# kakao/buffalo

Measured on NVIDIA H100. Metric: interactions/sec (nnz/s) ALS d=128, higher is better.
Workload: dtype f32

## Files before the change

### buffalo_b200/csrc/als_tc.cuh

```cuda
#pragma once
#include "als_generic.cuh"
#include "bfl_common.cuh"
#include <type_traits>

#include "sm90_ptx.cuh"

namespace bfl {
namespace tc {

using namespace sm90;

constexpr int N_CONV = 4, KH = N_CONV / 4;
constexpr int W_EPI = 0, W_MMA = 4, W_CONV = 8, W_PLAN = W_CONV + N_CONV;
constexpr int WARPS = 16, THREADS = WARPS * 32;
constexpr int REG_MMA = 200, REG_PLAN = 4 * 128 - 128 - 128 - REG_MMA;
constexpr int NXS = 8;
constexpr int PT = 2;
constexpr int NS = 3;
constexpr int GATHER_AHEAD = 1;
constexpr int NPG = 8, NP = NPG * PT;
constexpr int NBV = 8;
template <int D>
struct Cfg {
    static constexpr int TILE = D == 128 ? 32 : 16;
    static constexpr int NF = D / 128;
    static constexpr int LBO = D * 16;
    static constexpr int OP_BYTES = TILE * D * 2;
};
constexpr uint32_t F_FIRST = 1u << 8, F_LAST = 1u << 9, F_NEG = 1u << 10, F_STOP = 1u << 11;

__device__ __forceinline__ int msw(int c) { return ((c >> 1) & 3) << 3; }

constexpr int G_FLOATS = 16 * 17 / 2 * 64;
__device__ __forceinline__ int g_block(int R, int C) { return (R * (R + 1) / 2 + C) * 64; }

template <int D>
union Stage {
    unsigned char op[PT][2][Cfg<D>::OP_BYTES];
    float raw[PT][Cfg<D>::TILE * D];
};
static_assert(sizeof(Stage<128>::op) == sizeof(Stage<128>::raw) && sizeof(Stage<256>::op) == sizeof(Stage<256>::raw),
              "a group's rows and its slabs fill the same stage");

template <int D>
struct Smem {
    static constexpr int TILE = Cfg<D>::TILE;
    alignas(1024) Stage<D> st[NS];
    alignas(128) float mat[128 * 128];
    alignas(16) float g[G_FLOATS];
    alignas(16) float bvec[NBV][KH][D];
    alignas(16) float sumq[NBV][KH][D];
    alignas(16) float xs[NXS][D];
    alignas(16) float pv[4][32];
    alignas(16) float dl[4][32];
    alignas(16) float sws[NP][TILE];
    alignas(16) float wv[NP][TILE];
    alignas(16) int32_t keys[NP][TILE];
    float wsum[NBV][KH];
    uint32_t meta_raw[NP];
    uint32_t meta_op[NS][PT];
    int badrow[NXS];
    alignas(8) uint64_t plan_full[NPG], plan_empty[NPG], raw_full[NS], op_full[NS], st_empty[NS];
    alignas(8) uint64_t acc_full, acc_empty, x_full[NXS], d_full[4];
};
template <int D>
struct SmemDet : Smem<D> {
    double lossp[NXS][4][2];
};
static_assert(sizeof(SmemDet<128>) <= 232448 && sizeof(SmemDet<256>) <= 232448, "shared memory of als_tc_kernel");

struct TcArgs {
    AlsArgs a;
    const int32_t* items;
    float* scratch;
    int64_t split;
    int pass;
    int debug;
};

template <int D>
__host__ __device__ constexpr size_t scratch_floats() { return (size_t)D * D + 2 * D + 4; }

__global__ void tc_absmax_kernel(const float* __restrict__ p, size_t n, unsigned int* __restrict__ out) {
    float m = 0.f;
    const size_t gtid = (size_t)blockIdx.x * blockDim.x + threadIdx.x, gsz = (size_t)gridDim.x * blockDim.x;
    const size_t lead = min(n, (size_t)(((16 - ((uintptr_t)p & 15)) & 15) / 4));
    const size_t n4 = (n - lead) / 4;
    const float4* p4 = reinterpret_cast<const float4*>(p + lead);
    for (size_t i = gtid; i < n4; i += gsz) {
        const float4 v = __ldg(p4 + i);
        m = fmaxf(fmaxf(m, fmaxf(fabsf(v.x), fabsf(v.y))), fmaxf(fabsf(v.z), fabsf(v.w)));
    }
    for (size_t i = gtid; i < lead; i += gsz) m = fmaxf(m, fabsf(p[i]));
    for (size_t i = lead + n4 * 4 + gtid; i < n; i += gsz) m = fmaxf(m, fabsf(p[i]));
    for (int o = 16; o > 0; o >>= 1) m = fmaxf(m, __shfl_xor_sync(FULL, m, o));
    if ((threadIdx.x & 31) == 0 && m > 0.f) atomicMax(out, __float_as_uint(m));
}
__global__ void tc_scale_kernel(const unsigned int* __restrict__ ymax, const unsigned int* __restrict__ vmax, float alpha,
                                float* __restrict__ out) {
    const float y = __uint_as_float(*ymax), w = __uint_as_float(*vmax) * fabsf(alpha);
    const float top = y * sqrtf(w);
    int e = 0;
    if (top > 0.f && isfinite(top)) {
        int ex;
        frexpf(top, &ex);
        e = 15 - ex;
    }
    e = max(-60, min(60, e));
    out[0] = ldexpf(1.f, e);
    out[1] = ldexpf(1.f, -2 * e);
}

template <int D, bool PARTIAL, bool LOSS1, bool DET = false>
__global__ void __launch_bounds__(THREADS, 1) als_tc_kernel(TcArgs ta) {
    static_assert(D == 128 || (D == 256 && PARTIAL), "fused row solve: d = 128; split-row mode: d = 128 or 256");
    constexpr int TILE = Cfg<D>::TILE, NF = Cfg<D>::NF, LBO = Cfg<D>::LBO;
    extern __shared__ __align__(1024) unsigned char smem_raw_[];
    Smem<D>& S = *reinterpret_cast<Smem<D>*>(smem_raw_);
    [[maybe_unused]] SmemDet<D>& SD = *reinterpret_cast<SmemDet<D>*>(smem_raw_);
    const AlsArgs& a = ta.a;
    const int tid = threadIdx.x, lane = tid & 31;
    const int warp = __shfl_sync(FULL, tid >> 5, 0);

    if (tid == 0) {
        for (int i = 0; i < NS; ++i) {
            mbar_init(&S.raw_full[i], N_CONV);
            mbar_init(&S.op_full[i], N_CONV);
            mbar_init(&S.st_empty[i], 4);
        }
        for (int i = 0; i < NPG; ++i) {
            mbar_init(&S.plan_full[i], 1);
            mbar_init(&S.plan_empty[i], N_CONV);
        }
        mbar_init(&S.acc_full, 4);
        mbar_init(&S.acc_empty, 4);
        for (int b = 0; b < 4; ++b) mbar_init(&S.d_full[b], 1);
        for (int i = 0; i < NXS; ++i) {
            mbar_init(&S.x_full[i], 4);
            S.badrow[i] = 0;
        }
        mbar_init_fence();
    }
    const float scale = __ldg(a.tc_scales), inv2 = __ldg(a.tc_scales + 1);
    if (!PARTIAL) {
        const float s2 = scale * scale;
        const bool zero = ta.debug & 32;
        for (int e = tid; e < 128 * 128; e += THREADS) {
            const int r = e >> 7, c = e & 127;
            if ((r >> 3) >= (c >> 3)) {
                float g = zero ? 0.f : __ldg(a.G + e);
                g += r == c && !zero ? a.reg : 0.f;
                S.g[g_block(r >> 3, c >> 3) + 8 * (r & 7) + (c & 7)] = g * s2;
            }
        }
    }
    __syncthreads();

    const int64_t nitems = a.row_end - a.row_begin;
    const int64_t my_first = (int64_t)blockIdx.x;
    const int64_t stride = gridDim.x;

    auto item_info = [&](int64_t it, int& row, int64_t& beg, int64_t& n, int& slot) {
        if (PARTIAL) {
            const int32_t* p = ta.items + 3 * (a.row_begin + it);
            row = p[0];
            const int64_t rb = row == 0 ? 0 : a.indptr[row - 1];
            const int64_t rn = a.indptr[row] - rb;
            beg = rb + (int64_t)p[1] * ta.split;
            n = min(ta.split, rn - (int64_t)p[1] * ta.split);
            slot = DET ? (int)it : p[2];
        } else {
            row = a.row_list[a.row_begin + it];
            beg = row == 0 ? 0 : a.indptr[row - 1];
            n = a.indptr[row] - beg;
            slot = 0;
        }
    };

    if (warp >= W_PLAN) {
        setmaxnreg_dec<REG_PLAN>();
        if (warp != W_PLAN) return;
        uint32_t gsl = 0, rph = 0, pe = 0;
        auto tile_begin = [&]() -> uint32_t {
            if (pe == 0) mbar_wait_idle(&S.plan_empty[gsl], rph ^ 1u);
            return gsl * PT + pe;
        };
        auto tile_end = [&]() {
            if (++pe == PT) {
                if (lane == 0) mbar_arrive(&S.plan_full[gsl]);
                pe = 0;
                if (++gsl == NPG) { gsl = 0; rph ^= 1u; }
            }
        };
        auto emit = [&](unsigned mask, uint32_t flags, int32_t key, float w) {
            const int cnt = __popc(mask);
            const int slot = __popc(mask & ((1u << lane) - 1u));
            const uint32_t rs = tile_begin();
            if ((mask >> lane) & 1u) {
                S.keys[rs][slot] = key;
                S.sws[rs][slot] = sqrtf(fabsf(w)) * scale;
                S.wv[rs][slot] = w;
            } else {
                const int zslot = cnt + lane - slot;
                if (zslot < TILE) {
                    S.sws[rs][zslot] = 0.f;
                    S.wv[rs][zslot] = 0.f;
                }
            }
            if (lane == 0) S.meta_raw[rs] = (uint32_t)cnt | flags;
            __syncwarp();
            tile_end();
        };
        constexpr int SC = 4, SCN = SC * TILE;
        const bool inl = lane < TILE;
        auto load_id = [&](int64_t it, int& row, int& chunk) {
            row = -1;
            chunk = 0;
            if (it < nitems) {
                if (PARTIAL) {
                    const int32_t* p = ta.items + 3 * (a.row_begin + it);
                    row = p[0];
                    chunk = p[1];
                } else {
                    row = a.row_list[a.row_begin + it];
                }
            }
        };
        auto load_span = [&](int row, int chunk, const int32_t*& kp, const float*& vp, int& n) {
            kp = a.keys;
            vp = a.vals;
            n = 0;
            if (row >= 0) {
                const int64_t rb = row == 0 ? 0 : a.indptr[row - 1];
                const int64_t rn = a.indptr[row] - rb;
                int64_t beg = rb;
                n = (int)rn;
                if (PARTIAL) {
                    beg = rb + (int64_t)chunk * ta.split;
                    n = (int)min(ta.split, rn - (int64_t)chunk * ta.split);
                }
                kp = a.keys + (beg - a.shift);
                vp = a.vals + (beg - a.shift);
            }
        };
        auto load_sc = [&](const int32_t* kp, const float* vp, int n, int c0, int32_t (&key)[SC], float (&w)[SC]) {
#pragma unroll
            for (int s = 0; s < SC; ++s) {
                const int idx = c0 + s * TILE + lane;
                const bool ok = inl && idx < n;
                key[s] = ok ? kp[idx] : 0;
                w[s] = ok ? vp[idx] * a.alpha : 0.f;
            }
        };
        auto emit_sc = [&](int n, int c0, const int32_t (&key)[SC], const float (&w)[SC]) {
            bool neg = false;
#pragma unroll
            for (int s = 0; s < SC; ++s) neg |= w[s] < 0.f;
            if (!__any_sync(FULL, neg)) {
#pragma unroll
                for (int s = 0; s < SC; ++s) {
                    const int t0 = c0 + s * TILE;
                    if (t0 < n) {
                        const uint32_t meta = (uint32_t)min(TILE, n - t0) | (t0 == 0 ? F_FIRST : 0u) | (t0 + TILE >= n ? F_LAST : 0u);
                        const uint32_t rs = tile_begin();
                        if (inl) {
                            float sq;
                            asm("sqrt.approx.ftz.f32 %0, %1;" : "=f"(sq) : "f"(w[s]));
                            S.keys[rs][lane] = key[s];
                            S.sws[rs][lane] = sq * scale;
                            S.wv[rs][lane] = w[s];
                        }
                        if (lane == 0) S.meta_raw[rs] = meta;
                        __syncwarp();
                        tile_end();
                    }
                }
            } else {
#pragma unroll
                for (int s = 0; s < SC; ++s) {
                    const int t0 = c0 + s * TILE;
                    if (t0 < n) {
                        const bool valid = inl && t0 + lane < n;
                        const unsigned pm = __ballot_sync(FULL, valid && !(w[s] < 0.f));
                        const unsigned nm = __ballot_sync(FULL, valid && (w[s] < 0.f));
                        const bool lastc = t0 + TILE >= n;
                        uint32_t fl = (t0 == 0 ? F_FIRST : 0u);
                        if (pm) {
                            emit(pm, fl | ((lastc && !nm) ? F_LAST : 0u), key[s], w[s]);
                            fl = 0u;
                        }
                        if (nm) emit(nm, fl | F_NEG | (lastc ? F_LAST : 0u), key[s], w[s]);
                    }
                }
            }
        };
        const int32_t *kp0, *kp1, *kp2, *kp3;
        const float *vp0, *vp1, *vp2, *vp3;
        int n0, n1, n2, n3;
        int row_t, ch_t, row4, ch4;
        int32_t k0[SC], k1[SC], k2[SC], nk[SC];
        float w0[SC], w1[SC], w2[SC], nw[SC];
        load_id(my_first, row_t, ch_t);
        load_span(row_t, ch_t, kp0, vp0, n0);
        load_sc(kp0, vp0, n0, 0, k0, w0);
        load_id(my_first + stride, row_t, ch_t);
        load_span(row_t, ch_t, kp1, vp1, n1);
        load_sc(kp1, vp1, n1, 0, k1, w1);
        load_id(my_first + 2 * stride, row_t, ch_t);
        load_span(row_t, ch_t, kp2, vp2, n2);
        load_id(my_first + 3 * stride, row4, ch4);
        for (int64_t it = my_first; it < nitems; it += stride) {
            load_sc(kp2, vp2, n2, 0, k2, w2);
            load_span(row4, ch4, kp3, vp3, n3);
            load_id(it + 4 * stride, row4, ch4);
            for (int c0 = 0; c0 < n0; c0 += SCN) {
                const bool more = c0 + SCN < n0;
                if (more) load_sc(kp0, vp0, n0, c0 + SCN, nk, nw);
                emit_sc(n0, c0, k0, w0);
                if (more) {
#pragma unroll
                    for (int s = 0; s < SC; ++s) { k0[s] = nk[s]; w0[s] = nw[s]; }
                }
            }
#pragma unroll
            for (int s = 0; s < SC; ++s) { k0[s] = k1[s]; w0[s] = w1[s]; k1[s] = k2[s]; w1[s] = w2[s]; }
            kp0 = kp1; vp0 = vp1; n0 = n1; kp1 = kp2; vp1 = vp2; n1 = n2; kp2 = kp3; vp2 = vp3; n2 = n3;
        }
        do {
            const uint32_t rs = tile_begin();
            if (lane == 0) S.meta_raw[rs] = F_STOP;
            __syncwarp();
            tile_end();
        } while (pe != 0);
    } else if (warp >= W_MMA && warp < W_MMA + 4) {
        setmaxnreg_inc<REG_MMA>();
        const int r0 = (D == 256 && ta.pass == 2) ? 128 : 0, c0 = (D == 256 && ta.pass > 0) ? 128 : 0;
        const int wq = warp - W_MMA;
        const int fr = 16 * wq + (lane >> 2), fc = 2 * (lane & 3);
        constexpr int N0 = PARTIAL ? 128 : 64;
        float d0[N0 / 2], d1[64];
        auto mma0 = [&](auto neg, uint64_t adesc, uint64_t bdesc) {
            constexpr bool NEG = decltype(neg)::value;
            if constexpr (PARTIAL) wgmma_m64n128k16_f16<NEG>(d0, adesc, bdesc);
            else wgmma_m64n64k16_f16<NEG>(d0, adesc, bdesc);
        };
        const int rb = 2 * wq;
        const int g_lo = 8 * (lane >> 2) + fc, g_up = 8 * fc + (lane >> 2);
        auto g_pair = [&](int R, int C) -> float2 {
            const bool low = R >= C;
            const float* p = S.g + (low ? g_block(R, C) + g_lo : g_block(C, R) + g_up);
            return make_float2(p[0], p[low ? 1 : 8]);
        };
        auto acc_init_nh = [&](const int n, const int h) {
            if constexpr (PARTIAL) {
                d0[4 * n + 2 * h] = 0.f; d0[4 * n + 2 * h + 1] = 0.f;
                d1[4 * n + 2 * h] = 0.f; d1[4 * n + 2 * h + 1] = 0.f;
            } else {
                if (8 * n < N0) {
                    const float2 g0 = g_pair(rb + h, n);
                    d0[4 * n + 2 * h] = g0.x; d0[4 * n + 2 * h + 1] = g0.y;
                }
                const float2 g1 = n < 8 ? *reinterpret_cast<const float2*>(S.g + g_block(8 + rb + h, n) + g_lo)
                                        : g_pair(8 + rb + h, n);
                d1[4 * n + 2 * h] = g1.x; d1[4 * n + 2 * h + 1] = g1.y;
            }
        };
        auto acc_init = [&]() {
#pragma unroll
            for (int n = 0; n < 16; ++n)
#pragma unroll
                for (int h = 0; h < 2; ++h) acc_init_nh(n, h);
        };
        uint32_t os = 0, oph = 0, aph = 0;
        int64_t seq = 0;
        bool stop = false;
        acc_init();
        while (!stop) {
            mbar_wait(&S.op_full[os], oph);
            fence_proxy_async_smem();
#pragma unroll 1
            for (int e = 0; e < PT; ++e) {
                const uint32_t meta = S.meta_op[os][e];
                if (meta & F_STOP) {
                    stop = true;
                    break;
                }
                const int ksteps = (ta.debug & 2) ? 0 : (int)(meta & 0xffu);
                const uint32_t hi = s32(&S.st[os].op[e][0][0]), lo = s32(&S.st[os].op[e][1][0]);
                wgmma_fence();
#pragma unroll 1
                for (int ks = 0; ks < ksteps; ++ks) {
                    const uint32_t k0 = ks * 2 * LBO;
                    const uint64_t ah0 = smem_desc(hi + k0 + r0 * 16, LBO, 128), ah1 = smem_desc(hi + k0 + (r0 + 64) * 16, LBO, 128);
                    const uint64_t al0 = smem_desc(lo + k0 + r0 * 16, LBO, 128), al1 = smem_desc(lo + k0 + (r0 + 64) * 16, LBO, 128);
                    const uint64_t bh = smem_desc(hi + k0 + c0 * 16, LBO, 128), bl = smem_desc(lo + k0 + c0 * 16, LBO, 128);
                    if (meta & F_NEG) {
                        mma0(std::true_type{}, ah0, bh);
                        mma0(std::true_type{}, ah0, bl);
                        mma0(std::true_type{}, al0, bh);
                        wgmma_m64n128k16_f16<true>(d1, ah1, bh);
                        wgmma_m64n128k16_f16<true>(d1, ah1, bl);
                        wgmma_m64n128k16_f16<true>(d1, al1, bh);
                    } else {
                        mma0(std::false_type{}, ah0, bh);
                        mma0(std::false_type{}, ah0, bl);
                        mma0(std::false_type{}, al0, bh);
                        wgmma_m64n128k16_f16<false>(d1, ah1, bh);
                        wgmma_m64n128k16_f16<false>(d1, ah1, bl);
                        wgmma_m64n128k16_f16<false>(d1, al1, bh);
                    }
                }
                wgmma_commit();
                if (meta & F_LAST) {
                    wgmma_wait<0>();
#pragma unroll
                    for (int i = 0; i < 64; ++i) { if (i < N0 / 2) acc_fence(d0[i]); acc_fence(d1[i]); }
                    mbar_wait_idle(&S.acc_empty, aph ^ 1u);
                    if constexpr (PARTIAL) {
                        const int slot = DET ? (int)(my_first + seq * stride) : ta.items[3 * (a.row_begin + my_first + seq * stride) + 2];
                        float* sc = ta.scratch + (size_t)slot * scratch_floats<D>();
#pragma unroll
                        for (int n = 0; n < 16; ++n)
#pragma unroll
                            for (int h = 0; h < 2; ++h)
#pragma unroll
                                for (int i = 0; i < 2; ++i) {
                                    const int r = r0 + fr + 8 * h, c = c0 + 8 * n + fc + i;
                                    const float v0 = d0[4 * n + 2 * h + i] * inv2, v1 = d1[4 * n + 2 * h + i] * inv2;
                                    if constexpr (DET) {
                                        sc[(size_t)r * D + c] = v0;
                                        sc[(size_t)(r + 64) * D + c] = v1;
                                        if (r0 != c0) {
                                            sc[(size_t)c * D + r] = v0;
                                            sc[(size_t)c * D + r + 64] = v1;
                                        }
                                    } else {
                                        atomicAdd(sc + (size_t)r * D + c, v0);
                                        atomicAdd(sc + (size_t)(r + 64) * D + c, v1);
                                        if (r0 != c0) {
                                            atomicAdd(sc + (size_t)c * D + r, v0);
                                            atomicAdd(sc + (size_t)c * D + r + 64, v1);
                                        }
                                    }
                                }
                        acc_init();
                    } else {
#pragma unroll
                        for (int n = 0; n < 16; ++n)
#pragma unroll
                            for (int h = 0; h < 2; ++h) {
#pragma unroll
                                for (int i = 0; i < 2; ++i) {
                                    const int r = fr + 8 * h, c = 8 * n + fc + i;
                                    const float v1 = d1[4 * n + 2 * h + i] * inv2;
                                    S.mat[c * 128 + ((r + 64) ^ msw(c))] = v1;
                                    if (8 * n < N0) {
                                        S.mat[c * 128 + (r ^ msw(c))] = d0[4 * n + 2 * h + i] * inv2;
                                        S.mat[(r + 64) * 128 + (c ^ msw(r + 64))] = v1;
                                    }
                                }
                                acc_init_nh(n, h);
                            }
                    }
                    __syncwarp();
                    if (lane == 0) mbar_arrive(&S.acc_full);
                    aph ^= 1u;
                    ++seq;
                }
            }
            wgmma_wait<0>();
#pragma unroll
            for (int i = 0; i < 64; ++i) { if (i < N0 / 2) acc_fence(d0[i]); acc_fence(d1[i]); }
            __syncwarp();
            if (lane == 0) mbar_arrive(&S.st_empty[os]);
            if (++os == NS) { os = 0; oph ^= 1u; }
        }
    } else if (warp >= W_CONV && warp < W_CONV + N_CONV) {
        const int cta = tid - W_CONV * 32;
        const int ct = cta & 127;
        const int kh = cta >> 7;
        constexpr int CHS = TILE / 8 / KH;
        uint32_t rs = 0, rph = 0, bslot = 0;
        float2 bacc[NF], qacc[NF];
        float wacc = 0.f;
#pragma unroll
        for (int f = 0; f < NF; ++f) { bacc[f] = make_float2(0.f, 0.f); qacc[f] = make_float2(0.f, 0.f); }
        const int cw = cta >> 5;
        uint32_t gs = 0, gph = 0, grs = 0, grph = 0;
        bool plan_end = false;
        auto gather = [&]() {
            if (plan_end) {
                cp_async_commit();
                return;
            }
            mbar_wait(&S.plan_full[gs], gph);
            mbar_wait(&S.st_empty[grs], grph ^ 1u);
            const uint32_t gm0 = S.meta_raw[gs * PT], gm1 = S.meta_raw[gs * PT + 1];
            if (PT == 2 && !(ta.debug & 1) && ((gm0 | gm1) & F_STOP) == 0 && (gm0 & 0xffu) == TILE && (gm1 & 0xffu) == TILE) {
                int32_t kk[PT][TILE / N_CONV];
#pragma unroll
                for (int e = 0; e < PT; ++e)
#pragma unroll
                    for (int i = 0; i < TILE / N_CONV; ++i) kk[e][i] = S.keys[gs * PT + e][cw + N_CONV * i];
#pragma unroll
                for (int e = 0; e < PT; ++e)
#pragma unroll
                    for (int i = 0; i < TILE / N_CONV; ++i) {
                        const float* src = a.Y + (int64_t)kk[e][i] * a.ld + lane * 4;
                        float* dst = &S.st[grs].raw[e][(cw + N_CONV * i) * D + lane * 4];
#pragma unroll
                        for (int c = 0; c < D / 128; ++c) cp_async16_cg(dst + c * 128, src + c * 128);
                    }
            } else
#pragma unroll
            for (int e = 0; e < PT; ++e) {
                const uint32_t gmeta = S.meta_raw[gs * PT + e];
                if (gmeta & F_STOP) {
                    plan_end = true;
                } else {
                    const int gcnt = (ta.debug & 1) ? 0 : (int)(gmeta & 0xffu);
#pragma unroll
                    for (int i = 0; i < TILE / N_CONV; ++i) {
                        const int slot = cw + N_CONV * i;
                        if (slot < gcnt) {
                            const float* src = a.Y + (int64_t)S.keys[gs * PT + e][slot] * a.ld + lane * 4;
                            float* dst = &S.st[grs].raw[e][slot * D + lane * 4];
#pragma unroll
                            for (int c = 0; c < D / 128; ++c) cp_async16_cg(dst + c * 128, src + c * 128);
                        }
                    }
                }
            }
            cp_async_commit();
            if (++gs == NPG) { gs = 0; gph ^= 1u; }
            if (++grs == NS) { grs = 0; grph ^= 1u; }
        };
        uint32_t cs = 0;
        bool done = false;
        if (ta.debug & 16) {
            uint32_t ph = 0;
            for (;;) {
                mbar_wait(&S.plan_full[cs], ph);
                const bool stop = (S.meta_raw[cs * PT] | S.meta_raw[cs * PT + 1]) & F_STOP;
                __syncwarp();
                if (lane == 0) mbar_arrive(&S.plan_empty[cs]);
                if (stop) break;
                if (++cs == NPG) { cs = 0; ph ^= 1u; }
            }
            if (cta == 0) S.meta_op[0][0] = F_STOP;
            __syncwarp();
            if (lane == 0) mbar_arrive(&S.op_full[0]);
            done = true;
        }
#pragma unroll 1
        for (int i = 0; i < GATHER_AHEAD && !done; ++i) gather();
        while (!done) {
            gather();
            cp_async_wait_group<GATHER_AHEAD>();
            __syncwarp();
            if (lane == 0) mbar_arrive(&S.raw_full[rs]);
            mbar_wait(&S.raw_full[rs], rph);
            float qv[PT][CHS * 8 * NF];
#pragma unroll
            for (int e = 0; e < PT; ++e)
#pragma unroll
                for (int c = 0; c < CHS; ++c)
#pragma unroll
                    for (int i = 0; i < 8; ++i)
#pragma unroll
                        for (int f = 0; f < NF; ++f)
                            qv[e][(c * 8 + i) * NF + f] = S.st[rs].raw[e][((kh * CHS + c) * 8 + i) * D + ct + 128 * f];
            named_bar_sync(1, N_CONV * 32);
            const uint32_t cm0 = S.meta_raw[cs * PT], cm1 = S.meta_raw[cs * PT + 1];
            const bool fast2 = PT == 2 && !(ta.debug & 4) && ((cm0 | cm1) & F_STOP) == 0 && (cm0 & 0xffu) == TILE &&
                               (cm1 & 0xffu) == TILE;
            if (fast2) {
#pragma unroll
                for (int e = 0; e < PT; ++e) {
                    const uint32_t meta = e == 0 ? cm0 : cm1;
                    const uint32_t psl = cs * PT + e;
                    const bool first = (meta & F_FIRST) != 0;
#pragma unroll
                    for (int f = 0; f < NF; ++f) {
                        bacc[f].x = first ? 0.f : bacc[f].x; bacc[f].y = first ? 0.f : bacc[f].y;
                        qacc[f].x = first ? 0.f : qacc[f].x; qacc[f].y = first ? 0.f : qacc[f].y;
                    }
                    wacc = first ? 0.f : wacc;
                    unsigned char* hi = &S.st[rs].op[e][0][0];
                    unsigned char* lo = &S.st[rs].op[e][1][0];
#pragma unroll
                    for (int c = 0; c < CHS; ++c) {
                        const int kc = kh * CHS + c, k0 = kc * 8;
                        const float4 sa = *reinterpret_cast<const float4*>(&S.sws[psl][k0]);
                        const float4 sb = *reinterpret_cast<const float4*>(&S.sws[psl][k0 + 4]);
                        const float4 wa = *reinterpret_cast<const float4*>(&S.wv[psl][k0]);
                        const float4 wb = *reinterpret_cast<const float4*>(&S.wv[psl][k0 + 4]);
                        if (LOSS1) wacc += ((wa.x + wa.y) + (wa.z + wa.w)) + ((wb.x + wb.y) + (wb.z + wb.w));
#pragma unroll
                        for (int f = 0; f < NF; ++f) {
                            const int m = ct + 128 * f;
                            const float* q = &qv[e][0];
                            const float2 q01 = make_float2(q[(c * 8 + 0) * NF + f], q[(c * 8 + 1) * NF + f]);
                            const float2 q23 = make_float2(q[(c * 8 + 2) * NF + f], q[(c * 8 + 3) * NF + f]);
                            const float2 q45 = make_float2(q[(c * 8 + 4) * NF + f], q[(c * 8 + 5) * NF + f]);
                            const float2 q67 = make_float2(q[(c * 8 + 6) * NF + f], q[(c * 8 + 7) * NF + f]);
                            uint4 h4, l4;
                            split_f16x2(f2mul(q01, make_float2(sa.x, sa.y)), h4.x, l4.x);
                            split_f16x2(f2mul(q23, make_float2(sa.z, sa.w)), h4.y, l4.y);
                            split_f16x2(f2mul(q45, make_float2(sb.x, sb.y)), h4.z, l4.z);
                            split_f16x2(f2mul(q67, make_float2(sb.z, sb.w)), h4.w, l4.w);
                            const int off = kc * LBO + (m >> 3) * 128 + (m & 7) * 16;
                            *reinterpret_cast<uint4*>(hi + off) = h4;
                            *reinterpret_cast<uint4*>(lo + off) = l4;
                            bacc[f] = f2fma(make_float2(wa.x, wa.y), q01, bacc[f]);
                            bacc[f] = f2fma(make_float2(wa.z, wa.w), q23, bacc[f]);
                            bacc[f] = f2fma(make_float2(wb.x, wb.y), q45, bacc[f]);
                            bacc[f] = f2fma(make_float2(wb.z, wb.w), q67, bacc[f]);
                            if (LOSS1) {
                                qacc[f].x += (q01.x + q23.x) + (q45.x + q67.x);
                                qacc[f].y += (q01.y + q23.y) + (q45.y + q67.y);
                            }
                        }
                    }
#pragma unroll
                    for (int f = 0; f < NF; ++f) {
                        S.bvec[bslot][kh][ct + 128 * f] = bacc[f].x + bacc[f].y;
                        if (LOSS1) S.sumq[bslot][kh][ct + 128 * f] = qacc[f].x + qacc[f].y;
                    }
                    if (LOSS1 && ct == 0) S.wsum[bslot][kh] = wacc;
                    bslot = (bslot + ((meta & F_LAST) ? 1u : 0u)) & (NBV - 1);
                    if (cta == 0) S.meta_op[rs][e] = (uint32_t)(TILE / 16) | (meta & (F_FIRST | F_LAST | F_NEG));
                }
            } else
#pragma unroll
            for (int e = 0; e < PT; ++e) {
                if (done) continue;
                const uint32_t psl = cs * PT + e;
                const uint32_t meta = S.meta_raw[psl];
                if (meta & F_STOP) {
                    if (cta == 0) S.meta_op[rs][e] = F_STOP;
                    done = true;
                    continue;
                }
                const int cnt = (int)(meta & 0xffu), ksteps = (cnt + 15) >> 4;
                if (meta & F_FIRST) {
#pragma unroll
                    for (int f = 0; f < NF; ++f) { bacc[f] = make_float2(0.f, 0.f); qacc[f] = make_float2(0.f, 0.f); }
                    wacc = 0.f;
                }
                unsigned char* hi = &S.st[rs].op[e][0][0];
                unsigned char* lo = &S.st[rs].op[e][1][0];
                auto chunk = [&](auto guard, const int c) {
                    constexpr bool GUARD = decltype(guard)::value;
                    const int kc = kh * CHS + c, k0 = kc * 8;
                    const float4 sa = *reinterpret_cast<const float4*>(&S.sws[psl][k0]);
                    const float4 sb = *reinterpret_cast<const float4*>(&S.sws[psl][k0 + 4]);
                    const float4 wa = *reinterpret_cast<const float4*>(&S.wv[psl][k0]);
                    const float4 wb = *reinterpret_cast<const float4*>(&S.wv[psl][k0 + 4]);
                    if (LOSS1) wacc += ((wa.x + wa.y) + (wa.z + wa.w)) + ((wb.x + wb.y) + (wb.z + wb.w));
#pragma unroll
                    for (int f = 0; f < NF; ++f) {
                        const int m = ct + 128 * f;
                        float q[8];
#pragma unroll
                        for (int i = 0; i < 8; ++i) q[i] = qv[e][(c * 8 + i) * NF + f];
                        if (GUARD) {
#pragma unroll
                            for (int i = 0; i < 8; ++i) q[i] = (k0 + i < cnt) ? q[i] : 0.f;
                        }
                        const float2 q01 = make_float2(q[0], q[1]), q23 = make_float2(q[2], q[3]);
                        const float2 q45 = make_float2(q[4], q[5]), q67 = make_float2(q[6], q[7]);
                        uint4 h4, l4;
                        split_f16x2(f2mul(q01, make_float2(sa.x, sa.y)), h4.x, l4.x);
                        split_f16x2(f2mul(q23, make_float2(sa.z, sa.w)), h4.y, l4.y);
                        split_f16x2(f2mul(q45, make_float2(sb.x, sb.y)), h4.z, l4.z);
                        split_f16x2(f2mul(q67, make_float2(sb.z, sb.w)), h4.w, l4.w);
                        const int off = kc * LBO + (m >> 3) * 128 + (m & 7) * 16;
                        *reinterpret_cast<uint4*>(hi + off) = h4;
                        *reinterpret_cast<uint4*>(lo + off) = l4;
                        bacc[f] = f2fma(make_float2(wa.x, wa.y), q01, bacc[f]);
                        bacc[f] = f2fma(make_float2(wa.z, wa.w), q23, bacc[f]);
                        bacc[f] = f2fma(make_float2(wb.x, wb.y), q45, bacc[f]);
                        bacc[f] = f2fma(make_float2(wb.z, wb.w), q67, bacc[f]);
                        if (LOSS1) {
                            qacc[f].x += (q[0] + q[2]) + (q[4] + q[6]);
                            qacc[f].y += (q[1] + q[3]) + (q[5] + q[7]);
                        }
                    }
                };
                if (ta.debug & 4) {
                } else if (cnt == TILE) {
#pragma unroll
                    for (int c = 0; c < CHS; ++c) chunk(std::false_type{}, c);
                } else {
#pragma unroll
                    for (int c = 0; c < CHS; ++c)
                        if (kh * CHS + c < 2 * ksteps) chunk(std::true_type{}, c);
                }
                if (meta & F_LAST) {
#pragma unroll
                    for (int f = 0; f < NF; ++f) {
                        S.bvec[bslot][kh][ct + 128 * f] = bacc[f].x + bacc[f].y;
                        if (LOSS1) S.sumq[bslot][kh][ct + 128 * f] = qacc[f].x + qacc[f].y;
                    }
                    if (LOSS1 && ct == 0) S.wsum[bslot][kh] = wacc;
                    bslot = (bslot + 1) & (NBV - 1);
                }
                if (cta == 0) S.meta_op[rs][e] = (uint32_t)ksteps | (meta & (F_FIRST | F_LAST | F_NEG));
            }
            __syncwarp();
            if (lane == 0) {
                mbar_arrive(&S.plan_empty[cs]);
                mbar_arrive(&S.op_full[rs]);
            }
            cs = (cs + 1) & (NPG - 1);
            if (++rs == NS) { rs = 0; rph ^= 1u; }
        }
    } else {
        const int q = warp & 3;
        const int j = q * 32 + lane;
        float* pv = S.pv[q];
        double l_nume = 0.0, l_deno = 0.0;
        const float tol = a.tol;
        if constexpr (PARTIAL) {
            int row = 0, slot = 0, nrow = 0, nslot = 0;
            int64_t beg, n = 0, nbeg, nn = 0;
            if (my_first < nitems) item_info(my_first, row, beg, n, slot);
            for (int64_t seq = 0; my_first + seq * stride < nitems; ++seq) {
                const int64_t nit = my_first + (seq + 1) * stride;
                if (nit < nitems) item_info(nit, nrow, nbeg, nn, nslot);
                const uint32_t aph = (uint32_t)(seq & 1);
                const uint32_t bs = (uint32_t)(seq & (NBV - 1));
                mbar_wait_idle(&S.acc_full, aph);
                float* sc = ta.scratch + (size_t)slot * scratch_floats<D>();
                if constexpr (DET) {
                    if (ta.pass == 0) {
                        for (int jj = j; jj < D; jj += 128) {
                            sc[(size_t)D * D + jj] = S.bvec[bs][0][jj] + (KH == 2 ? S.bvec[bs][KH - 1][jj] : 0.f);
                            if (LOSS1) sc[(size_t)D * D + D + jj] = S.sumq[bs][0][jj] + (KH == 2 ? S.sumq[bs][KH - 1][jj] : 0.f);
                        }
                        if (LOSS1 && j < 4)
                            sc[(size_t)D * D + 2 * D + j] = j == 0 ? S.wsum[bs][0] + (KH == 2 ? S.wsum[bs][KH - 1] : 0.f) : 0.f;
                    }
                } else if (ta.pass == 0) {
                    for (int jj = j; jj < D; jj += 128) {
                        atomicAdd(sc + (size_t)D * D + jj, S.bvec[bs][0][jj] + (KH == 2 ? S.bvec[bs][KH - 1][jj] : 0.f));
                        if (LOSS1) atomicAdd(sc + (size_t)D * D + D + jj, S.sumq[bs][0][jj] + (KH == 2 ? S.sumq[bs][KH - 1][jj] : 0.f));
                    }
                    if (LOSS1 && j == 0) atomicAdd(sc + (size_t)D * D + 2 * D, S.wsum[bs][0] + (KH == 2 ? S.wsum[bs][KH - 1] : 0.f));
                }
                __syncwarp();
                if (lane == 0) mbar_arrive(&S.acc_empty);
                row = nrow; slot = nslot; n = nn;
            }
        } else {
            auto row_of = [&](int64_t sq) -> int {
                const int64_t it = my_first + sq * stride;
                return it < nitems ? a.row_list[a.row_begin + it] : -1;
            };
            auto len_of = [&](int row) -> float {
                if (row < 0 || !a.compute_loss) return 0.f;
                return (float)(a.indptr[row] - (row == 0 ? 0 : a.indptr[row - 1]));
            };
            int row = (ta.debug & 16) ? -1 : row_of(0), row1 = row_of(1), row2 = row_of(2);
            float xj = row >= 0 ? a.X[(int64_t)row * a.ld + j] : 0.f;
            float x1 = row1 >= 0 ? a.X[(int64_t)row1 * a.ld + j] : 0.f;
            float nlen = len_of(row), nlen1 = len_of(row1);
            if (row >= 0) {
                S.xs[0][j] = xj;
                __syncwarp();
                if (lane == 0) mbar_arrive(&S.x_full[0]);
            }
            auto mat = [&](int c) -> float { return S.mat[c * 128 + (j ^ msw(c))]; };
            for (int64_t seq = 0; row >= 0; ++seq) {
                const int row3 = row_of(seq + 3);
                const float x2 = row2 >= 0 ? a.X[(int64_t)row2 * a.ld + j] : 0.f;
                const float nlen2 = len_of(row2);
                if (row1 >= 0) {
                    S.xs[(seq + 1) & (NXS - 1)][j] = x1;
                    __syncwarp();
                    if (lane == 0) mbar_arrive(&S.x_full[(seq + 1) & (NXS - 1)]);
                }
                const uint32_t aph = (uint32_t)(seq & 1);
                const uint32_t bs = (uint32_t)(seq & (NBV - 1));
                const uint32_t xsl = (uint32_t)(seq & (NXS - 1));
                const float* xs = S.xs[xsl];
                mbar_wait(&S.x_full[xsl], (uint32_t)((seq / NXS) & 1));
                mbar_wait_idle(&S.acc_full, aph);
                if (ta.debug & 8) {
                    __syncwarp();
                    if (lane == 0) mbar_arrive(&S.acc_empty);
                    row = row1; row1 = row2; row2 = row3;
                    xj = x1; x1 = x2;
                    continue;
                }
                const float bj = S.bvec[bs][0][j] + (KH == 2 ? S.bvec[bs][KH - 1][j] : 0.f);
                double ln_row = 0.0, ld_row = 0.0;
                float hM = 0.f;
                float md[32];
#pragma unroll
                for (int c = 0; c < D / 32; ++c) {
                    float h0 = 0.f, h1 = 0.f;
#pragma unroll
                    for (int i = 0; i < 32; i += 4) {
                        const float4 x4 = *reinterpret_cast<const float4*>(xs + c * 32 + i);
                        const float m0 = mat(c * 32 + i), m1 = mat(c * 32 + i + 1), m2 = mat(c * 32 + i + 2), m3 = mat(c * 32 + i + 3);
                        h0 = fmaf(m0, x4.x, h0); h1 = fmaf(m1, x4.y, h1);
                        h0 = fmaf(m2, x4.z, h0); h1 = fmaf(m3, x4.w, h1);
                        if (c == q) { md[i] = m0; md[i + 1] = m1; md[i + 2] = m2; md[i + 3] = m3; }
                    }
                    hM += h0 + h1;
                }
                if (a.compute_loss) {
                    const float kappa = a.adaptive_reg ? nlen : 1.0f;
                    double t = (double)(kappa * a.reg * xj * xj);
                    if (a.axis == 1) {
                        t += (double)xj * (double)hM - (double)(a.reg * xj * xj) -
                             2.0 * (double)xj * ((double)bj + (double)S.sumq[bs][0][j] + (KH == 2 ? (double)S.sumq[bs][KH - 1][j] : 0.0));
                        if (j == 0) {
                            const double ws = (double)S.wsum[bs][0] + (KH == 2 ? (double)S.wsum[bs][KH - 1] : 0.0);
                            t += (double)nlen + ws;
                            l_deno += (double)a.Y_rows + ws;
                        }
                    }
                    if constexpr (DET) {
                        ln_row = warp_sum_d(t);
                        ld_row = l_deno;
                        l_deno = 0.0;
                        if (q < 3 && lane == 0) {
                            SD.lossp[xsl][q][0] = ln_row;
                            SD.lossp[xsl][q][1] = ld_row;
                        }
                    } else {
                        l_nume += t;
                    }
                }
                float h = hM - bj;
#pragma unroll 1
                for (int B = 0; B < q; ++B) {
                    float mv[32];
#pragma unroll
                    for (int i = 0; i < 32; ++i) mv[i] = mat(B * 32 + i);
                    mbar_wait(&S.d_full[B], aph);
                    float u0 = 0.f, u1 = 0.f;
#pragma unroll
                    for (int i = 0; i < 32; i += 4) {
                        const float4 d4 = *reinterpret_cast<const float4*>(&S.dl[B][i]);
                        u0 = fmaf(mv[i], d4.x, u0);
                        u1 = fmaf(mv[i + 1], d4.y, u1);
                        u0 = fmaf(mv[i + 2], d4.z, u0);
                        u1 = fmaf(mv[i + 3], d4.w, u1);
                    }
                    h -= u0 + u1;
                }
                if constexpr (DET) {
                    if (q == 3 && lane == 0 && a.loss && a.compute_loss) {
                        double sn = SD.lossp[xsl][0][0], sd = SD.lossp[xsl][0][1];
#pragma unroll
                        for (int w = 1; w < 3; ++w) {
                            sn += SD.lossp[xsl][w][0];
                            sd += SD.lossp[xsl][w][1];
                        }
                        a.loss[2 * (int64_t)row] = sn + ln_row;
                        a.loss[2 * (int64_t)row + 1] = sd + ld_row;
                    }
                }
                __syncwarp();
                if (lane == 0) mbar_arrive(&S.acc_empty);
                float xv = 0.f;
                {
                    float r = h, p = h;
                    float rsold = warp_sum(r * r);
                    bool act = rsold > tol;
#pragma unroll 1
                    for (int step = 0; step < 3; ++step) {
                        pv[lane] = p;
                        __syncwarp();
                        float a0 = 0.f, a1 = 0.f, a2 = 0.f, a3 = 0.f;
#pragma unroll
                        for (int i = 0; i < 32; i += 4) {
                            const float4 p4 = *reinterpret_cast<const float4*>(pv + i);
                            a0 = fmaf(md[i], p4.x, a0); a1 = fmaf(md[i + 1], p4.y, a1);
                            a2 = fmaf(md[i + 2], p4.z, a2); a3 = fmaf(md[i + 3], p4.w, a3);
                        }
                        __syncwarp();
                        const float Ap = (a0 + a1) + (a2 + a3);
                        const float pAp = warp_sum(p * Ap);
                        const float ss = act ? __fdividef(rsold, pAp) : 0.f;
                        xv = fmaf(ss, p, xv);
                        r = fmaf(-ss, Ap, r);
                        const float rsnew = warp_sum(r * r);
                        act = act && !(rsnew < tol);
                        if (act) p = fmaf(__fdividef(rsnew, rsold), p, r);
                        rsold = act ? rsnew : rsold;
                    }
                }
                float v = xj - xv;
                const bool badw = __any_sync(FULL, !isfinite(v));
                a.X[(int64_t)row * a.ld + j] = v;
                for (int pr = 0; pr < a.n_peer; ++pr) a.peerX[pr][(int64_t)row * a.ld + j] = v;
                if (q < 3) {
                    S.dl[q][lane] = xv;
                    if (badw && lane == 0) atomicOr(&S.badrow[xsl], 1);
                    __syncwarp();
                    if (lane == 0) mbar_arrive(&S.d_full[q]);
                }
                if (q == 3) {
                    const bool bad = badw || (S.badrow[xsl] != 0);
                    if (bad) {
#pragma unroll
                        for (int c = 0; c < 4; ++c) {
                            a.X[(int64_t)row * a.ld + c * 32 + lane] = 0.f;
                            for (int pr = 0; pr < a.n_peer; ++pr) a.peerX[pr][(int64_t)row * a.ld + c * 32 + lane] = 0.f;
                        }
                        __syncwarp();
                        if (lane == 0) S.badrow[xsl] = 0;
                    }
                }
                row = row1; row1 = row2; row2 = row3;
                xj = x1; x1 = x2;
                nlen = nlen1; nlen1 = nlen2;
            }
            if (!DET && a.loss && a.compute_loss) {
                l_nume = warp_sum_d(l_nume);
                l_deno = warp_sum_d(l_deno);
                if (lane == 0 && (l_nume != 0.0 || l_deno != 0.0)) {
                    atomicAdd(a.loss, l_nume);
                    atomicAdd(a.loss + 1, l_deno);
                }
            }
        }
    }
}

inline bool tc_applicable(int optimizer_code, int d, int vdim, int block_size) {
    return optimizer_code == 8 && d == 128 && vdim == 128 && block_size == 32;
}
inline bool tc_split_applicable(int optimizer_code, int d, int vdim, int block_size) {
    return optimizer_code == 8 && (d == 128 || d == 256) && vdim == d && block_size == 32;
}

inline int tc_note_absmax(const float* p, size_t n, unsigned int* out, int num_sms, cudaStream_t st) {
    BFL_CUDA(cudaMemsetAsync(out, 0, sizeof(unsigned int), st));
    if (n == 0) return BFL_OK;
    const int grid = (int)std::min<size_t>((n / 4 + 255) / 256 + 1, (size_t)num_sms * 8);
    tc_absmax_kernel<<<grid, 256, 0, st>>>(p, n, out);
    BFL_LAUNCHED();
    return BFL_OK;
}
inline int tc_update_scale(const unsigned int* ymax, const unsigned int* vmax, float alpha, float* scales, cudaStream_t st) {
    tc_scale_kernel<<<1, 1, 0, st>>>(ymax, vmax, alpha, scales);
    BFL_LAUNCHED();
    return BFL_OK;
}

__global__ void tc_count_items_kernel(const int64_t* __restrict__ indptr, const int32_t* __restrict__ list, int64_t nrows,
                                      int64_t split, unsigned long long* total) {
    for (int64_t i = (int64_t)blockIdx.x * blockDim.x + threadIdx.x; i < nrows; i += (int64_t)gridDim.x * blockDim.x) {
        const int row = list[i];
        const int64_t n = indptr[row] - (row == 0 ? 0 : indptr[row - 1]);
        atomicAdd(total, (unsigned long long)((n + split - 1) / split));
    }
}
__global__ void tc_fill_items_kernel(const int64_t* __restrict__ indptr, const int32_t* __restrict__ list, int64_t nrows,
                                     int64_t split, unsigned long long* cursor, int32_t* __restrict__ items) {
    for (int64_t i = (int64_t)blockIdx.x * blockDim.x + threadIdx.x; i < nrows; i += (int64_t)gridDim.x * blockDim.x) {
        const int row = list[i];
        const int64_t n = indptr[row] - (row == 0 ? 0 : indptr[row - 1]);
        const int64_t nc = (n + split - 1) / split;
        const unsigned long long pos = atomicAdd(cursor, (unsigned long long)nc);
        for (int64_t c = 0; c < nc; ++c) {
            items[3 * (pos + c) + 0] = row;
            items[3 * (pos + c) + 1] = (int32_t)c;
            items[3 * (pos + c) + 2] = (int32_t)i;
        }
    }
}

__global__ void tc_chunk_counts_kernel(const int64_t* __restrict__ indptr, const int32_t* __restrict__ list, int64_t nrows,
                                       int64_t split, long long* __restrict__ counts) {
    for (int64_t i = (int64_t)blockIdx.x * blockDim.x + threadIdx.x; i < nrows; i += (int64_t)gridDim.x * blockDim.x) {
        const int row = list[i];
        const int64_t n = indptr[row] - (row == 0 ? 0 : indptr[row - 1]);
        counts[i] = (n + split - 1) / split;
    }
}
__global__ void tc_fill_items_scanned_kernel(const int32_t* __restrict__ list, int64_t nrows,
                                             const long long* __restrict__ chunk_end, int32_t* __restrict__ items) {
    for (int64_t i = (int64_t)blockIdx.x * blockDim.x + threadIdx.x; i < nrows; i += (int64_t)gridDim.x * blockDim.x) {
        const int64_t pos = i == 0 ? 0 : chunk_end[i - 1], nc = chunk_end[i] - pos;
        for (int64_t c = 0; c < nc; ++c) {
            items[3 * (pos + c) + 0] = list[i];
            items[3 * (pos + c) + 1] = (int32_t)c;
            items[3 * (pos + c) + 2] = (int32_t)i;
        }
    }
}

__global__ void __launch_bounds__(256) tc_chunk_reduce_kernel(const float* __restrict__ chunks, const long long* __restrict__ chunk_end,
                                                              int64_t row0, int64_t chunk0, size_t slot_floats, int nf4,
                                                              float* __restrict__ rows_out) {
    const int64_t i = row0 + blockIdx.y;
    const int64_t c0 = (i == 0 ? 0 : chunk_end[i - 1]) - chunk0, c1 = chunk_end[i] - chunk0;
    float4* out = reinterpret_cast<float4*>(rows_out + (size_t)blockIdx.y * slot_floats);
    for (int e = blockIdx.x * blockDim.x + threadIdx.x; e < nf4; e += gridDim.x * blockDim.x) {
        float4 acc = __ldg(reinterpret_cast<const float4*>(chunks + (size_t)c0 * slot_floats) + e);
        for (int64_t c = c0 + 1; c < c1; ++c) {
            const float4 v = __ldg(reinterpret_cast<const float4*>(chunks + (size_t)c * slot_floats) + e);
            acc.x = __fadd_rn(acc.x, v.x);
            acc.y = __fadd_rn(acc.y, v.y);
            acc.z = __fadd_rn(acc.z, v.z);
            acc.w = __fadd_rn(acc.w, v.w);
        }
        out[e] = acc;
    }
}

template <int D>
int tc_launch_partial(const AlsArgs& a, const int32_t* items, int64_t nitems, float* scratch, int64_t nslots,
                      int64_t split, int num_sms, cudaStream_t st, bool det = false) {
    if (nitems <= 0) return BFL_OK;
    if (!a.tc_scales) BFL_FAIL(BFL_ERR_STATE, "tensor-core ALS kernel: operand scale not prepared");
    TcArgs ta;
    ta.a = a;
    ta.a.row_begin = 0;
    ta.a.row_end = nitems;
    ta.items = items;
    ta.scratch = scratch;
    ta.split = split;
    ta.debug = 0;
    if (!det) BFL_CUDA(cudaMemsetAsync(scratch, 0, sizeof(float) * scratch_floats<D>() * (size_t)nslots, st));
    const size_t smem = sizeof(Smem<D>);
    const int grid = (int)std::min<int64_t>(nitems, (int64_t)num_sms);
    for (ta.pass = 0; ta.pass < (D == 128 ? 1 : 3); ++ta.pass) {
        if (det && a.compute_loss && a.axis == 1) {
            BFL_CUDA(cudaFuncSetAttribute(als_tc_kernel<D, true, true, true>, cudaFuncAttributeMaxDynamicSharedMemorySize, (int)smem));
            als_tc_kernel<D, true, true, true><<<grid, THREADS, smem, st>>>(ta);
        } else if (det) {
            BFL_CUDA(cudaFuncSetAttribute(als_tc_kernel<D, true, false, true>, cudaFuncAttributeMaxDynamicSharedMemorySize, (int)smem));
            als_tc_kernel<D, true, false, true><<<grid, THREADS, smem, st>>>(ta);
        } else if (a.compute_loss && a.axis == 1) {
            BFL_CUDA(cudaFuncSetAttribute(als_tc_kernel<D, true, true>, cudaFuncAttributeMaxDynamicSharedMemorySize, (int)smem));
            als_tc_kernel<D, true, true><<<grid, THREADS, smem, st>>>(ta);
        } else {
            BFL_CUDA(cudaFuncSetAttribute(als_tc_kernel<D, true, false>, cudaFuncAttributeMaxDynamicSharedMemorySize, (int)smem));
            als_tc_kernel<D, true, false><<<grid, THREADS, smem, st>>>(ta);
        }
        BFL_LAUNCHED();
    }
    return BFL_OK;
}

inline int tc_launch(const AlsArgs& a, int num_sms, cudaStream_t st, bool det_loss = false) {
    const int64_t nrows = a.row_end - a.row_begin;
    if (nrows <= 0) return BFL_OK;
    if (!a.tc_scales) BFL_FAIL(BFL_ERR_STATE, "tensor-core ALS kernel: operand scale not prepared");
    TcArgs ta;
    ta.a = a;
    ta.items = nullptr;
    ta.scratch = nullptr;
    ta.split = 0;
    ta.pass = 0;
    ta.debug = getenv("BFL_TC_DEBUG") ? atoi(getenv("BFL_TC_DEBUG")) : 0;
    const size_t smem = sizeof(Smem<128>);
    const int grid = (int)std::min<int64_t>(nrows, (int64_t)num_sms);
    if (det_loss) {
        const size_t smem_det = sizeof(SmemDet<128>);
        if (a.axis == 1) {
            BFL_CUDA(cudaFuncSetAttribute(als_tc_kernel<128, false, true, true>, cudaFuncAttributeMaxDynamicSharedMemorySize, (int)smem_det));
            als_tc_kernel<128, false, true, true><<<grid, THREADS, smem_det, st>>>(ta);
        } else {
            BFL_CUDA(cudaFuncSetAttribute(als_tc_kernel<128, false, false, true>, cudaFuncAttributeMaxDynamicSharedMemorySize, (int)smem_det));
            als_tc_kernel<128, false, false, true><<<grid, THREADS, smem_det, st>>>(ta);
        }
    } else if (a.compute_loss && a.axis == 1) {
        BFL_CUDA(cudaFuncSetAttribute(als_tc_kernel<128, false, true>, cudaFuncAttributeMaxDynamicSharedMemorySize, (int)smem));
        als_tc_kernel<128, false, true><<<grid, THREADS, smem, st>>>(ta);
    } else {
        BFL_CUDA(cudaFuncSetAttribute(als_tc_kernel<128, false, false>, cudaFuncAttributeMaxDynamicSharedMemorySize, (int)smem));
        als_tc_kernel<128, false, false><<<grid, THREADS, smem, st>>>(ta);
    }
    BFL_LAUNCHED();
    return BFL_OK;
}

}
}
```

Measured before the change: 1.532 billion.

## Store Gram matrix as packed lower-triangle blocks and release accumulator earlier

```diff
diff --git a/buffalo_b200/csrc/als_tc.cuh b/buffalo_b200/csrc/als_tc.cuh
--- a/buffalo_b200/csrc/als_tc.cuh
+++ b/buffalo_b200/csrc/als_tc.cuh
@@ -29,7 +29,9 @@
 };
 constexpr uint32_t F_FIRST = 1u << 8, F_LAST = 1u << 9, F_NEG = 1u << 10, F_STOP = 1u << 11;
 
+constexpr int MAT_BLOCK = 32 * 33, MAT_FLOATS = 4 * 5 / 2 * MAT_BLOCK;
 __device__ __forceinline__ int msw(int c) { return ((c >> 1) & 3) << 3; }
+__device__ __forceinline__ int mat_block(int R, int C) { return (R * (R + 1) / 2 + C) * MAT_BLOCK; }
 
 constexpr int G_FLOATS = 16 * 17 / 2 * 64;
 __device__ __forceinline__ int g_block(int R, int C) { return (R * (R + 1) / 2 + C) * 64; }
@@ -46,13 +48,14 @@
 struct Smem {
     static constexpr int TILE = Cfg<D>::TILE;
     alignas(1024) Stage<D> st[NS];
-    alignas(128) float mat[128 * 128];
+    alignas(128) float mat[MAT_FLOATS];
     alignas(16) float g[G_FLOATS];
     alignas(16) float bvec[NBV][KH][D];
     alignas(16) float sumq[NBV][KH][D];
     alignas(16) float xs[NXS][D];
     alignas(16) float pv[4][32];
-    alignas(16) float dl[4][32];
+    alignas(16) float dl[2][4][32];
+    alignas(16) float fold[6][32 * 32];
     alignas(16) float sws[NP][TILE];
     alignas(16) float wv[NP][TILE];
     alignas(16) int32_t keys[NP][TILE];
@@ -61,7 +64,7 @@
     uint32_t meta_op[NS][PT];
     int badrow[NXS];
     alignas(8) uint64_t plan_full[NPG], plan_empty[NPG], raw_full[NS], op_full[NS], st_empty[NS];
-    alignas(8) uint64_t acc_full, acc_empty, x_full[NXS], d_full[4];
+    alignas(8) uint64_t acc_full, acc_empty, x_full[NXS], d_full[2][4];
 };
 template <int D>
 struct SmemDet : Smem<D> {
@@ -134,7 +137,7 @@
         }
         mbar_init(&S.acc_full, 4);
         mbar_init(&S.acc_empty, 4);
-        for (int b = 0; b < 4; ++b) mbar_init(&S.d_full[b], 1);
+        for (int b = 0; b < 8; ++b) mbar_init(&S.d_full[b >> 2][b & 3], 1);
         for (int i = 0; i < NXS; ++i) {
             mbar_init(&S.x_full[i], 4);
             S.badrow[i] = 0;
@@ -445,19 +448,19 @@
                                 }
                         acc_init();
                     } else {
+                        const int hb = wq >> 1;
+                        float* const m0 = S.mat + mat_block(hb, 0) + 33 * fc;
+                        float* const m1 = S.mat + mat_block(2 + hb, 0) + 33 * fc;
+                        const int xe = (fr & 31) ^ msw(fc);
 #pragma unroll
                         for (int n = 0; n < 16; ++n)
 #pragma unroll
                             for (int h = 0; h < 2; ++h) {
 #pragma unroll
                                 for (int i = 0; i < 2; ++i) {
-                                    const int r = fr + 8 * h, c = 8 * n + fc + i;
-                                    const float v1 = d1[4 * n + 2 * h + i] * inv2;
-                                    S.mat[c * 128 + ((r + 64) ^ msw(c))] = v1;
-                                    if (8 * n < N0) {
-                                        S.mat[c * 128 + (r ^ msw(c))] = d0[4 * n + 2 * h + i] * inv2;
-                                        S.mat[(r + 64) * 128 + (c ^ msw(r + 64))] = v1;
-                                    }
+                                    const int C = n >> 2, e = 33 * (8 * (n & 3) + i) + (xe ^ (8 * h));
+                                    if (C < 3 || hb == 1) m1[MAT_BLOCK * C + e] = d1[4 * n + 2 * h + i] * inv2;
+                                    if (8 * n < N0 && (C == 0 || hb == 1)) m0[MAT_BLOCK * C + e] = d0[4 * n + 2 * h + i] * inv2;
                                 }
                                 acc_init_nh(n, h);
                             }
@@ -771,7 +774,11 @@
                 __syncwarp();
                 if (lane == 0) mbar_arrive(&S.x_full[0]);
             }
-            auto mat = [&](int c) -> float { return S.mat[c * 128 + (j ^ msw(c))]; };
+            const float* const mrow = S.mat + mat_block(q, 0);
+            const int ml = msw(lane);
+            float* const pan = S.fold[q * (q - 1) / 2] + lane;
+            auto mat_lo = [&](int C, int i) -> float { return mrow[MAT_BLOCK * C + 33 * i + (lane ^ msw(i))]; };
+            auto mat_up = [&](int C, int i) -> float { return S.mat[mat_block(C, q) + 33 * lane + (i & 7) + ((i & 24) ^ ml)]; };
             for (int64_t seq = 0; row >= 0; ++seq) {
                 const int row3 = row_of(seq + 3);
                 const float x2 = row2 >= 0 ? a.X[(int64_t)row2 * a.ld + j] : 0.f;
@@ -785,6 +792,7 @@
                 const uint32_t bs = (uint32_t)(seq & (NBV - 1));
                 const uint32_t xsl = (uint32_t)(seq & (NXS - 1));
                 const float* xs = S.xs[xsl];
+                const uint32_t dsl = (uint32_t)(seq & 1), dph = (uint32_t)((seq >> 1) & 1);
                 mbar_wait(&S.x_full[xsl], (uint32_t)((seq / NXS) & 1));
                 mbar_wait_idle(&S.acc_full, aph);
                 if (ta.debug & 8) {
@@ -798,19 +806,32 @@
                 double ln_row = 0.0, ld_row = 0.0;
                 float hM = 0.f;
                 float md[32];
-#pragma unroll
-                for (int c = 0; c < D / 32; ++c) {
+                auto hblock = [&](const int c, auto mat, auto keep) {
                     float h0 = 0.f, h1 = 0.f;
 #pragma unroll
                     for (int i = 0; i < 32; i += 4) {
                         const float4 x4 = *reinterpret_cast<const float4*>(xs + c * 32 + i);
-                        const float m0 = mat(c * 32 + i), m1 = mat(c * 32 + i + 1), m2 = mat(c * 32 + i + 2), m3 = mat(c * 32 + i + 3);
+                        const float m0 = mat(i), m1 = mat(i + 1), m2 = mat(i + 2), m3 = mat(i + 3);
                         h0 = fmaf(m0, x4.x, h0); h1 = fmaf(m1, x4.y, h1);
                         h0 = fmaf(m2, x4.z, h0); h1 = fmaf(m3, x4.w, h1);
-                        if (c == q) { md[i] = m0; md[i + 1] = m1; md[i + 2] = m2; md[i + 3] = m3; }
+                        keep(i, m0, m1, m2, m3);
                     }
                     hM += h0 + h1;
-                }
+                };
+#pragma unroll 1
+                for (int c = 0; c < q; ++c)
+                    hblock(c, [&](int i) { return mat_lo(c, i); }, [&](int i, float m0, float m1, float m2, float m3) {
+                        float* pp = pan + 1024 * c + 32 * i;
+                        pp[0] = m0; pp[32] = m1; pp[64] = m2; pp[96] = m3;
+                    });
+                hblock(q, [&](int i) { return mat_lo(q, i); }, [&](int i, float m0, float m1, float m2, float m3) {
+                    md[i] = m0; md[i + 1] = m1; md[i + 2] = m2; md[i + 3] = m3;
+                });
+#pragma unroll 1
+                for (int c = q + 1; c < D / 32; ++c)
+                    hblock(c, [&](int i) { return mat_up(c, i); }, [](int, float, float, float, float) {});
+                __syncwarp();
+                if (lane == 0) mbar_arrive(&S.acc_empty);
                 if (a.compute_loss) {
                     const float kappa = a.adaptive_reg ? nlen : 1.0f;
                     double t = (double)(kappa * a.reg * xj * xj);
@@ -840,12 +861,12 @@
                 for (int B = 0; B < q; ++B) {
                     float mv[32];
 #pragma unroll
-                    for (int i = 0; i < 32; ++i) mv[i] = mat(B * 32 + i);
-                    mbar_wait(&S.d_full[B], aph);
+                    for (int i = 0; i < 32; ++i) mv[i] = pan[1024 * B + 32 * i];
+                    mbar_wait(&S.d_full[dsl][B], dph);
                     float u0 = 0.f, u1 = 0.f;
 #pragma unroll
                     for (int i = 0; i < 32; i += 4) {
-                        const float4 d4 = *reinterpret_cast<const float4*>(&S.dl[B][i]);
+                        const float4 d4 = *reinterpret_cast<const float4*>(&S.dl[dsl][B][i]);
                         u0 = fmaf(mv[i], d4.x, u0);
                         u1 = fmaf(mv[i + 1], d4.y, u1);
                         u0 = fmaf(mv[i + 2], d4.z, u0);
@@ -865,8 +886,6 @@
                         a.loss[2 * (int64_t)row + 1] = sd + ld_row;
                     }
                 }
-                __syncwarp();
-                if (lane == 0) mbar_arrive(&S.acc_empty);
                 float xv = 0.f;
                 {
                     float r = h, p = h;
@@ -900,10 +919,10 @@
                 a.X[(int64_t)row * a.ld + j] = v;
                 for (int pr = 0; pr < a.n_peer; ++pr) a.peerX[pr][(int64_t)row * a.ld + j] = v;
                 if (q < 3) {
-                    S.dl[q][lane] = xv;
+                    S.dl[dsl][q][lane] = xv;
                     if (badw && lane == 0) atomicOr(&S.badrow[xsl], 1);
                     __syncwarp();
-                    if (lane == 0) mbar_arrive(&S.d_full[q]);
+                    if (lane == 0) mbar_arrive(&S.d_full[dsl][q]);
                 }
                 if (q == 3) {
                     const bool bad = badw || (S.badrow[xsl] != 0);
```

Result: faster. 1.558 billion, median of 6 (+1.7%).
